# SimLeek/pySILEnT

Hardware: AMD Instinct MI355X
Metric: Mpx/s full pyramid line-end pass @1080p, 1/2/4/8 GPU; % HBM roofline (higher is better)
Workload: dtype f32

## Files before the change

### pysilent_amd/csrc/silent_rgb2.h

```cpp
#pragma once

#include "silent_rgb.h"

namespace silent {

typedef float f2 __attribute__((ext_vector_type(2)));
typedef unsigned long long u64;
typedef const __attribute__((address_space(4))) u64* ku64_p;

constexpr int kRgb2Halo = 8;
constexpr int kRgb2Cols = 128 - 2 * kRgb2Halo;
#ifndef RGB2_WAVES
#define RGB2_WAVES 2
#endif
constexpr int kRgb2Waves = RGB2_WAVES;
constexpr int kRgb2TW = kRgb2Waves * kRgb2Cols;
constexpr int kRgb2RowHalo = 7;
#ifndef RGB2_STORE_AUX
#define RGB2_STORE_AUX 2
#endif
constexpr int kRgb2StoreAux = RGB2_STORE_AUX;
constexpr int kRgb2Out = 0x40000000;

constexpr int kRgb2Blk = 16;
constexpr int kRgb2StreamMax = SILENT_RGB_STREAM_MAX;

constexpr int rgb2_popc(unsigned v) { return v ? (int)(v & 1u) + rgb2_popc(v >> 1) : 0; }

struct RgbSym {
    float rgc[12];
    float rgby[27];
};
constexpr int kSymRgc = 12, kSymRgby = 27, kSymStripe = 48;

template <unsigned RGC_PAIRS, bool STRIPE_SUM, bool RGBY_TWO, bool END_TWO, bool SYM = false>
struct Rgb2Layout {
    static constexpr int n_rgc = SYM ? kSymRgc : 9 * rgb2_popc(RGC_PAIRS & 0x1ffu);
    static constexpr int n_rgby = SYM ? kSymRgby : RGBY_TWO ? 45 : 81;
    static constexpr int n_stripe = SYM ? kSymStripe : STRIPE_SUM ? 27 : 81;
    static constexpr bool blur_sym = RGBY_TWO && END_TWO;
    static constexpr int n_blur = blur_sym ? 16 : 49;
    static constexpr int n_end = END_TWO ? 45 : 81;
    static constexpr int b_rgc = 0, b_rgby = b_rgc + n_rgc, b_stripe = (b_rgby + n_rgby + (SYM ? 1 : 0)) & ~(SYM ? 1 : 0),
                         b_blur = b_stripe + n_stripe, b_end = b_blur + n_blur, total = b_end + n_end;
    static constexpr int blocks = ((total + 2 * kRgb2Blk - 1) / (2 * kRgb2Blk)) * 2;
    static_assert(!SYM || (STRIPE_SUM && RGBY_TWO && END_TWO), "the symmetric forms extend the two-group instantiation");
};

constexpr int rgb2_conv_pos(unsigned pairs, int o, int dy, int dx, int i) {
    const unsigned row = (pairs >> (o * 3)) & 7u;
    const int before = 9 * rgb2_popc(pairs & ((1u << (o * 3)) - 1u));
    const int rank = dx * rgb2_popc(row) + rgb2_popc(row & ((1u << i) - 1u));
    return before + rank * 3 + (2 - dy);
}
inline int rgb2_fill_stream(const RgbW& w, unsigned rgc_pairs, bool stripe_sum, bool rgby_two, bool end_two, float* out,
                            const RgbSym* sym = nullptr) {
    const bool blur_sym = rgby_two && end_two;
    int n = 0;
    auto conv = [&](const float* k, unsigned pairs) {
        const int base = n;
        for (int o = 0; o < 3; ++o)
            for (int dy = 0; dy < 3; ++dy)
                for (int dx = 0; dx < 3; ++dx)
                    for (int i = 0; i < 3; ++i)
                        if ((pairs >> (o * 3 + i)) & 1u) {
                            out[base + rgb2_conv_pos(pairs, o, dy, dx, i)] = k[((o * 3 + dy) * 3 + dx) * 3 + i];
                            ++n;
                        }
    };
    auto two = [&](const float* k) {
        for (int j = 0; j < 9; ++j)
            for (int dy = 0; dy < 3; ++dy) out[n + j * 3 + (2 - dy)] = k[dy * 9 + j];
        for (int t = 0; t < 18; ++t) out[n + 27 + t] = k[27 + t];
        n += 45;
    };
    if (sym) {
        for (int c = 0; c < 3; ++c) {
            out[n + 0 + c] = sym->rgc[c * 4 + 0];
            out[n + 3 + c] = sym->rgc[c * 4 + 2];
            out[n + 6 + c] = sym->rgc[c * 4 + 1];
            out[n + 9 + c] = sym->rgc[c * 4 + 3];
        }
        n += kSymRgc;
        for (int t = 0; t < 9; ++t) out[n + t] = sym->rgby[t];
        for (int o = 0; o < 3; ++o) {
            out[n + 9 + o] = sym->rgby[9 + 0];
            out[n + 12 + o] = sym->rgby[9 + 3];
            out[n + 15 + o] = sym->rgby[9 + 1];
        }
        for (int t = 0; t < 9; ++t) out[n + 18 + t] = sym->rgby[18 + t];
        n += kSymRgby;
        if (n & 1) out[n++] = 0.0f;
        for (int o = 0; o < 3; ++o) {
            for (int dy = 0; dy < 3; ++dy) {
                const float l = w.stripe[((o * 3 + dy) * 3 + 0) * 3], c = w.stripe[((o * 3 + dy) * 3 + 1) * 3], r = w.stripe[((o * 3 + dy) * 3 + 2) * 3];
                out[n + (2 - dy) * 2] = l;
                out[n + (2 - dy) * 2 + 1] = r;
                out[n + 6 + (2 - dy)] = c;
                out[n + 10 + (2 - dy) * 2] = r;
                out[n + 10 + (2 - dy) * 2 + 1] = l;
            }
            out[n + 9] = 0.0f;
            n += 16;
        }
    } else {
    conv(w.rgc, rgc_pairs & 0x1ffu);
    if (rgby_two) two(w.rgby);
    else conv(w.rgby, 0x1ffu);
    if (stripe_sum) {
        for (int o = 0; o < 3; ++o)
            for (int dx = 0; dx < 3; ++dx)
                for (int dy = 0; dy < 3; ++dy) out[n + o * 9 + dx * 3 + (2 - dy)] = w.stripe[((o * 3 + dy) * 3 + dx) * 3];
        n += 27;
    } else {
        conv(w.stripe, 0x1ffu);
    }
    }
    if (blur_sym) {
        for (int j = 0; j < 4; ++j)
            for (int d = 0; d < 4; ++d) out[n + j * 4 + d] = w.blur[(3 + d) * 7 + j];
        n += 16;
    } else {
        for (int dx = 0; dx < 7; ++dx)
            for (int k = 0; k < 7; ++k) out[n + dx * 7 + k] = w.blur[(6 - k) * 7 + dx];
        n += 49;
    }
    if (end_two) two(w.end);
    else conv(w.end, 0x1ffu);
    const int total = n;
    while (n % (2 * kRgb2Blk)) out[n++] = 0.0f;
    return total;
}

struct Rgb2Args {
    const float* pyr;
    float* orient_out;
    float* line_out;
    float* value_out;
    LevelTab tab;
    RgbP prm;
    int th;
    unsigned* mm;
    float* sum;
    int* nan_flags;
    long long sum_frame;
    long long sum_off[kMaxLevels];
    alignas(64) float ws[kRgb2StreamMax];
};
static_assert(offsetof(Rgb2Args, ws) % 64 == 0, "weight blocks are whole 64-byte lines of the kernarg segment");

template <int NP>
struct WPairs {
    u64 p[NP];
};
__device__ __forceinline__ void wait_weights() { __builtin_amdgcn_s_waitcnt(0xC07F); }

template <int NB>
struct WStream {
    WPairs<kRgb2Blk / 2> A, B;
    ku64_p wp;
    template <int BLK>
    __device__ __forceinline__ void request() {
        ku64_p q = wp;
        __builtin_amdgcn_sched_barrier(0);
        asm volatile("" : "+s"(q));
        if constexpr (BLK & 1) {
#pragma unroll
            for (int k = 0; k < kRgb2Blk / 2; ++k) B.p[k] = q[BLK * (kRgb2Blk / 2) + k];
        } else {
#pragma unroll
            for (int k = 0; k < kRgb2Blk / 2; ++k) A.p[k] = q[BLK * (kRgb2Blk / 2) + k];
        }
    }
    template <int IDX>
    __device__ __forceinline__ u64 pair() {
        constexpr int blk = IDX / kRgb2Blk;
        if constexpr (IDX % kRgb2Blk == 0) {
            wait_weights();
            request<(blk + 1) % NB>();
        }
        if constexpr (blk & 1) return B.p[(IDX % kRgb2Blk) / 2];
        else return A.p[(IDX % kRgb2Blk) / 2];
    }
    template <int IDX>
    __device__ __forceinline__ f2 fma(const f2& x, const f2& c) {
        const u64 w = pair<IDX>();
        f2 r;
        if constexpr ((IDX & 1) == 0) asm volatile("v_pk_fma_f32 %0, %1, %2, %3 op_sel_hi:[1,0,1]" : "=v"(r) : "v"(x), "s"(w), "v"(c));
        else asm volatile("v_pk_fma_f32 %0, %1, %2, %3 op_sel:[0,1,0] op_sel_hi:[1,1,1]" : "=v"(r) : "v"(x), "s"(w), "v"(c));
        return r;
    }
    template <int IDX>
    __device__ __forceinline__ f2 fma0(const f2& x) {
        const u64 w = pair<IDX>();
        f2 r;
        if constexpr ((IDX & 1) == 0) asm volatile("v_pk_fma_f32 %0, %1, %2, 0 op_sel_hi:[1,0,0]" : "=v"(r) : "v"(x), "s"(w));
        else asm volatile("v_pk_fma_f32 %0, %1, %2, 0 op_sel:[0,1,0] op_sel_hi:[1,1,0]" : "=v"(r) : "v"(x), "s"(w));
        return r;
    }
    template <int IDX>
    __device__ __forceinline__ f2 mul(const f2& x) {
        const u64 w = pair<IDX>();
        f2 r;
        if constexpr ((IDX & 1) == 0) asm volatile("v_pk_mul_f32 %0, %1, %2 op_sel_hi:[1,0]" : "=v"(r) : "v"(x), "s"(w));
        else asm volatile("v_pk_mul_f32 %0, %1, %2 op_sel:[0,1] op_sel_hi:[1,1]" : "=v"(r) : "v"(x), "s"(w));
        return r;
    }
    template <int IDX>
    __device__ __forceinline__ f2 fma_sw(const f2& x, const f2& c) {
        static_assert((IDX & 1) == 0, "an aligned SGPR pair");
        const u64 w = pair<IDX>();
        f2 r;
        asm volatile("v_pk_fma_f32 %0, %1, %2, %3 op_sel:[1,0,0] op_sel_hi:[0,1,1]" : "=v"(r) : "v"(x), "s"(w), "v"(c));
        return r;
    }
    template <int IDX>
    __device__ __forceinline__ f2 fma0_sw(const f2& x) {
        static_assert((IDX & 1) == 0, "an aligned SGPR pair");
        const u64 w = pair<IDX>();
        f2 r;
        asm volatile("v_pk_fma_f32 %0, %1, %2, 0 op_sel:[1,0,0] op_sel_hi:[0,1,0]" : "=v"(r) : "v"(x), "s"(w));
        return r;
    }
    template <int FROM, int TO>
    __device__ __forceinline__ void skip() {
        if constexpr (FROM < TO) {
            constexpr int nb = (FROM + kRgb2Blk - 1) / kRgb2Blk * kRgb2Blk;
            if constexpr (nb < TO) {
                (void)pair<nb>();
                skip<nb + 1, TO>();
            }
        }
    }
};

template <int I>
using ic = std::integral_constant<int, I>;
template <int B, int E, class F>
__device__ __forceinline__ void rgb2_for(F&& f) {
    if constexpr (B < E) {
        f(ic<B>{});
        rgb2_for<B + 1, E>(f);
    }
}

__device__ __forceinline__ void neighbours2(const f2& c, f2& l, f2& r) {
    l.x = from_lane_below(c.y);
    l.y = c.x;
    r.x = c.y;
    r.y = from_lane_above(c.x);
}

__device__ __forceinline__ f2 side_pair(const f2& c) { return f2{from_lane_above(c.x), from_lane_below(c.y)}; }
__device__ __forceinline__ f2 pk_add_swap_both(const f2& a, const f2& b) {
    f2 r;
    asm("v_pk_add_f32 %0, %1, %2 op_sel:[1,1] op_sel_hi:[0,0]" : "=v"(r) : "v"(a), "v"(b));
    return r;
}
__device__ __forceinline__ f2 pk_add_swap_second(const f2& a, const f2& b) {
    f2 r;
    asm("v_pk_add_f32 %0, %1, %2 op_sel:[0,1] op_sel_hi:[1,0]" : "=v"(r) : "v"(a), "v"(b));
    return r;
}
__device__ __forceinline__ float relu_clip_max3(float v, float hi) {
    float r;
    asm("v_maximum3_f32 %0, %1, 0, 0" : "=v"(r) : "v"(v));
    asm("v_minimum3_f32 %0, %1, %2, %2" : "=v"(r) : "v"(r), "s"(hi));
    return r;
}

template <unsigned PAIRS, int BASE, class WS>
__device__ __forceinline__ void conv3_roll2(const f2 (&v)[3][3], WS& ws, f2 (&pa)[3], f2 (&pb)[3], f2 (&done)[3]) {
    f2 npa[3], npb[3];
    rgb2_for<0, 3>([&](auto oo) {
        constexpr int o = decltype(oo)::value;
        constexpr unsigned row = (PAIRS >> (o * 3)) & 7u;
        f2 t2 = pa[o], t1 = pb[o], t0 = f2{0.0f, 0.0f};
        if constexpr (row != 0) {
            constexpr int first_i = (row & 1u) ? 0 : ((row & 2u) ? 1 : 2);
            rgb2_for<0, 9>([&](auto jj) {
                constexpr int j = decltype(jj)::value, dx = j / 3, i = j % 3;
                if constexpr ((row >> i) & 1u) {
                    constexpr int p2 = BASE + rgb2_conv_pos(PAIRS, o, 2, dx, i);
                    t2 = ws.template fma<p2>(v[dx][i], t2);
                    t1 = ws.template fma<p2 + 1>(v[dx][i], t1);
                    if constexpr (dx == 0 && i == first_i) t0 = ws.template fma0<p2 + 2>(v[dx][i]);
                    else t0 = ws.template fma<p2 + 2>(v[dx][i], t0);
                }
            });
        }
        done[o] = t2;
        npa[o] = t1;
        npb[o] = t0;
    });
#pragma unroll
    for (int o = 0; o < 3; ++o) {
        pa[o] = npa[o];
        pb[o] = npb[o];
    }
}

template <unsigned M0, unsigned M1, unsigned M2, int BASE, class WS>
__device__ __forceinline__ void conv3_roll2_struct(const f2 (&v)[3][3], WS& ws, f2 (&pa)[6], f2 (&pb)[6], f2 (&done)[3]) {
    constexpr unsigned M[3] = {M0, M1, M2};
    f2 acc2[6], acc1[6], acc0[6];
#pragma unroll
    for (int q = 0; q < 6; ++q) {
        acc2[q] = pa[q];
        acc1[q] = pb[q];
        acc0[q] = f2{0.0f, 0.0f};
    }
    rgb2_for<0, 9>([&](auto jj) {
        constexpr int j = decltype(jj)::value, dx = j / 3, i = j % 3;
        constexpr int p = BASE + j * 3;
        constexpr int q2 = ((M[i] >> (2 * 3 + dx)) & 1u) ? i : 3 + i;
        constexpr int q1 = ((M[i] >> (1 * 3 + dx)) & 1u) ? i : 3 + i;
        constexpr bool a0 = (M[i] >> dx) & 1u;
        constexpr int q0 = a0 ? i : 3 + i;
        acc2[q2] = ws.template fma<p>(v[dx][i], acc2[q2]);
        acc1[q1] = ws.template fma<p + 1>(v[dx][i], acc1[q1]);
        constexpr unsigned taps = M[i] & 7u;
        constexpr bool seen = (dx >= 1 && (((taps >> 0) & 1u) != 0) == a0) || (dx >= 2 && (((taps >> 1) & 1u) != 0) == a0);
        if constexpr (!seen) acc0[q0] = ws.template fma0<p + 2>(v[dx][i]);
        else acc0[q0] = ws.template fma<p + 2>(v[dx][i], acc0[q0]);
    });
    {
        constexpr int PM = BASE + 27;
        f2 t[3];
        rgb2_for<0, 3>([&](auto oo) {
            constexpr int o = decltype(oo)::value;
            t[o] = ws.template mul<PM + o>(acc2[0]);
        });
        rgb2_for<1, 6>([&](auto kk) {
            constexpr int k = decltype(kk)::value;
            rgb2_for<0, 3>([&](auto oo) {
                constexpr int o = decltype(oo)::value;
                t[o] = ws.template fma<PM + k * 3 + o>(acc2[k], t[o]);
            });
        });
#pragma unroll
        for (int o = 0; o < 3; ++o) done[o] = t[o];
    }
#pragma unroll
    for (int q = 0; q < 6; ++q) {
        pa[q] = acc1[q];
        pb[q] = acc0[q];
    }
}

template <int BASE, class WS>
__device__ __forceinline__ void conv3_roll2_sum(const f2 (&s)[3], WS& ws, f2 (&pa)[3], f2 (&pb)[3], f2 (&done)[3]) {
    f2 npa[3], npb[3];
    rgb2_for<0, 3>([&](auto oo) {
        constexpr int o = decltype(oo)::value;
        f2 t2 = pa[o], t1 = pb[o], t0;
        rgb2_for<0, 3>([&](auto xx) {
            constexpr int dx = decltype(xx)::value, p = BASE + o * 9 + dx * 3;
            t2 = ws.template fma<p>(s[dx], t2);
            t1 = ws.template fma<p + 1>(s[dx], t1);
            if constexpr (dx == 0) t0 = ws.template fma0<p + 2>(s[dx]);
            else t0 = ws.template fma<p + 2>(s[dx], t0);
        });
        done[o] = t2;
        npa[o] = t1;
        npb[o] = t0;
    });
#pragma unroll
    for (int o = 0; o < 3; ++o) {
        pa[o] = npa[o];
        pb[o] = npb[o];
    }
}

__device__ __forceinline__ float relu_ok(float v, bool ok) { return ok ? relu_tf(v) : 0.0f; }
__device__ __forceinline__ float relu_max3(float v) {
    float r;
    asm("v_maximum3_f32 %0, %1, 0, 0" : "=v"(r) : "v"(v));
    return r;
}
__device__ __forceinline__ float relu_max3_poisoned(float v, float u) {
    float r;
    asm("v_maximum3_f32 %0, %1, 0, %2" : "=v"(r) : "v"(v), "v"(u));
    return r;
}

typedef _Float16 rgb_half;
template <unsigned RGC_PAIRS, bool STRIPE_SUM, unsigned RGBY_A, unsigned END_A0, unsigned END_A1, unsigned END_A2, bool MM = false, bool SYM = false,
          bool ST4 = false, typename ST = float>
__global__ __launch_bounds__(64 * kRgb2Waves) __attribute__((amdgpu_waves_per_eu((MM || ST4) ? 3 : 4, 8))) void rgb_line_end2_kernel(const Rgb2Args args) {
    typedef Rgb2Layout<RGC_PAIRS, STRIPE_SUM, RGBY_A != kDense, END_A0 != kDense, SYM> L;
    constexpr bool kHalf = std::is_same<ST, rgb_half>::value;
    static_assert(kHalf || std::is_same<ST, float>::value, "orient / line_end are stored as float32 or float16");
    static_assert(!(kHalf && ST4), "ST4 is a float32 store form");
    static_assert(L::blocks * kRgb2Blk <= kRgb2StreamMax, "stream fits its kernarg array");
    static_assert((RGC_PAIRS & 0x1ffu) == 0x1ffu || (RGC_PAIRS & 0x1ffu) == 0x111u, "rgc: dense or channel-diagonal");
    constexpr bool kRgcDiag = (RGC_PAIRS & 0x1ffu) == 0x111u;
    const int R = args.th, NROWS = R + 2 * kRgb2RowHalo;
    const float* __restrict__ pyr = args.pyr;
    float* __restrict__ orient_out = args.orient_out;
    float* __restrict__ line_out = args.line_out;
    float* __restrict__ value_out = args.value_out;
    const LevelTab& tab = args.tab;
    const RgbP& prm = args.prm;

    typedef const __attribute__((address_space(4))) char* kchar_p;
    WStream<L::blocks> ws;
    ws.wp = (ku64_p)((kchar_p)__builtin_amdgcn_kernarg_segment_ptr() + offsetof(Rgb2Args, ws));
    ws.template request<0>();

    const TileCoord tc = locate_tile(tab, blockIdx.x);
    const int H = tab.h[tc.level], W = tab.w[tc.level];
    const long long base_px = (long long)tc.frame * tab.frame_px + tab.px_off[tc.level];
    const float* __restrict__ src = pyr + base_px * 3;
    const int lane = threadIdx.x & 63;
    const int wave = __builtin_amdgcn_readfirstlane(threadIdx.x >> 6);
    const int xw0 = tc.tx * kRgb2TW + wave * kRgb2Cols;
    if (xw0 >= W) return;
    const int y0 = tc.ty * R;
    const int x0 = xw0 + 2 * lane - kRgb2Halo, x1 = x0 + 1;
    const bool col0 = x0 >= 0 && x0 < W, col1 = x1 >= 0 && x1 < W;
    const bool out_lane = lane >= kRgb2Halo / 2 && lane < 64 - kRgb2Halo / 2;
    const bool out0 = out_lane && x0 < W, out1 = out_lane && x1 < W;
    const int rb = W * 12;
    const int rows_t = R < H - y0 ? R : H - y0;
    const unsigned lvl_bytes = (unsigned)H * (unsigned)rb;
    const unsigned tile_bytes = (unsigned)rows_t * (unsigned)rb;
    const long long tile_px = base_px + (long long)y0 * W;
    const __amdgpu_buffer_rsrc_t r_src = __builtin_amdgcn_make_buffer_rsrc((void*)src, 0, lvl_bytes, 0x00020000);
    __amdgpu_buffer_rsrc_t r_orient = __builtin_amdgcn_make_buffer_rsrc((void*)(orient_out + tile_px * 3), 0, orient_out ? tile_bytes : 0u, 0x00020000);
    __amdgpu_buffer_rsrc_t r_line = __builtin_amdgcn_make_buffer_rsrc((void*)(line_out + tile_px * 3), 0, line_out ? tile_bytes : 0u, 0x00020000);
    unsigned mis_o = 0, mis_l = 0;
    if constexpr (kHalf) {
        auto half_rsrc = [&](float* p, unsigned& mis) {
            const unsigned long long b = reinterpret_cast<unsigned long long>(p) + (unsigned long long)(tile_px * 6);
            mis = (unsigned)__builtin_amdgcn_readfirstlane((int)(b & 2ull));
            return __builtin_amdgcn_make_buffer_rsrc((void*)(b - mis), 0, p ? tile_bytes / 2u + mis : 0u, 0x00020000);
        };
        r_orient = half_rsrc(orient_out, mis_o);
        r_line = half_rsrc(line_out, mis_l);
    }
    const __amdgpu_buffer_rsrc_t r_value = __builtin_amdgcn_make_buffer_rsrc((void*)(value_out + tile_px), 0, value_out ? tile_bytes / 3u : 0u, 0x00020000);
    const int in0 = col0 ? x0 * 12 : kRgb2Out, in1 = col1 ? x1 * 12 : kRgb2Out;
    const int xa = xw0 - kRgb2Halo + lane, xb = xa + 64;
    const int sta = (lane >= kRgb2Halo && xa < W) ? xa * 12 : kRgb2Out, stb = (lane < 64 - kRgb2Halo && xb < W) ? xb * 12 : kRgb2Out;
    const int sv2 = (out0 && out1) ? x0 * 4 : kRgb2Out, sv1 = (out0 && !out1) ? x0 * 4 : kRgb2Out;
    const bool padc0 = x0 >= prm.pad && x0 < W - prm.pad, padc1 = x1 >= prm.pad && x1 < W - prm.pad;
    const f2 inv3p = {1.0f / 3.0f, 1.0f / 3.0f};
    const f2 zero2 = {0.0f, 0.0f};

    f2 a1[3] = {zero2, zero2, zero2}, b1[3] = {zero2, zero2, zero2};
    f2 a2[6] = {zero2, zero2, zero2, zero2, zero2, zero2}, b2[6] = {zero2, zero2, zero2, zero2, zero2, zero2};
    f2 a3[3] = {zero2, zero2, zero2}, b3[3] = {zero2, zero2, zero2};
    f2 a5[6] = {zero2, zero2, zero2, zero2, zero2, zero2}, b5[6] = {zero2, zero2, zero2, zero2, zero2, zero2};
    f2 pb[7] = {zero2, zero2, zero2, zero2, zero2, zero2, zero2};
    __shared__ f2 s_hist[kRgb2Waves][4][3][64];
    float mm_mx = kPoolLowest, mm_nmn = kPoolLowest;
    float mm_grp = kPoolLowest;
    unsigned long long mm_nan = 0;
    const int gpt = (R + kSumRows - 1) / kSumRows, nxp = (W + 1) >> 1;
    const unsigned sum_bytes = (MM && args.sum) ? (unsigned)((rows_t + kSumRows - 1) / kSumRows) * (unsigned)nxp * 4u : 0u;
    const __amdgpu_buffer_rsrc_t r_sum = __builtin_amdgcn_make_buffer_rsrc(
        (void*)(args.sum + (long long)tc.frame * args.sum_frame + args.sum_off[tc.level] + (long long)tc.ty * gpt * nxp), 0, sum_bytes, 0x00020000);
    const int ssum = out0 ? (x0 >> 1) * 4 : kRgb2Out;
    __shared__ __attribute__((aligned(16))) float s_tr[kRgb2Waves][ST4 ? 4 * 384 : kHalf ? 1 : 384];
    float* const tr = s_tr[wave];
    typedef int i3 __attribute__((ext_vector_type(3)));
    f2* const tr_in = reinterpret_cast<f2*>(tr) + lane * 3;
    const float* const tr_out = tr + (lane >> 1) * 6 + (lane & 1);
    auto store_row3 = [&](const f2 (&val)[3], __amdgpu_buffer_rsrc_t rsrc, int ro) {
#pragma unroll
        for (int c = 0; c < 3; ++c) tr_in[c] = val[c];
        const i3 da = {__float_as_int(tr_out[0]), __float_as_int(tr_out[2]), __float_as_int(tr_out[4])};
        const i3 db = {__float_as_int(tr_out[192]), __float_as_int(tr_out[194]), __float_as_int(tr_out[196])};
        __builtin_amdgcn_raw_buffer_store_b96(da, rsrc, (int)((unsigned)sta + (unsigned)ro), 0, kRgb2StoreAux);
        __builtin_amdgcn_raw_buffer_store_b96(db, rsrc, (int)((unsigned)stb + (unsigned)ro), 0, kRgb2StoreAux);
    };
    const int hb = x0 * 6;
    const bool h_two = out0 && out1, h_one = out0 && !out1;
    const bool h_next = lane + 1 < 64 - kRgb2Halo / 2 && x0 + 2 < W;
    const bool h_lead = lane == kRgb2Halo / 2 - 1;
    const int he96 = h_two ? hb : kRgb2Out, ho96 = (h_two && h_next) ? hb + 2 : kRgb2Out;
    const int ho64 = (h_two && !h_next) ? hb + 2 : kRgb2Out;
    const int h32 = h_one ? hb : kRgb2Out;
    const int he16 = h_one ? hb + 4 : kRgb2Out;
    const int ho16 = h_lead ? hb + 12 : (h_two && !h_next) ? hb + 10 : kRgb2Out;
    const unsigned lead_sh = h_lead ? 16u : 0u;
    auto store_row3h = [&](const f2 (&val)[3], __amdgpu_buffer_rsrc_t rsrc, unsigned ro) {
        typedef rgb_half h2 __attribute__((ext_vector_type(2)));
        typedef int i2h __attribute__((ext_vector_type(2)));
        const int d0 = __builtin_bit_cast(int, h2{(rgb_half)val[0].x, (rgb_half)val[1].x});
        const int d1 = __builtin_bit_cast(int, h2{(rgb_half)val[2].x, (rgb_half)val[0].y});
        const int d2 = __builtin_bit_cast(int, h2{(rgb_half)val[1].y, (rgb_half)val[2].y});
        int m = -(int)((ro >> 1) & 1u);
        asm volatile("" : "+s"(m));
        auto pick = [&](int even, int odd) { return (odd & m) | (even & ~m); };
        const unsigned sh = (unsigned)(m & 16);
        const int up = __builtin_amdgcn_update_dpp(0, d0, 0x130 , 0xf, 0xf, true);
        const int e0 = (int)__builtin_amdgcn_alignbit((unsigned)d1, (unsigned)d0, sh);
        const int e1 = (int)__builtin_amdgcn_alignbit((unsigned)d2, (unsigned)d1, sh);
        const int e2 = (int)__builtin_amdgcn_alignbit((unsigned)up, (unsigned)d2, sh);
        const int last = pick(e1, (int)((unsigned)e2 >> lead_sh));
        __builtin_amdgcn_raw_buffer_store_b96(i3{e0, e1, e2}, rsrc, (int)((unsigned)pick(he96, ho96) + ro), 0, kRgb2StoreAux);
        __builtin_amdgcn_raw_buffer_store_b64(i2h{e0, e1}, rsrc, (int)((unsigned)pick(kRgb2Out, ho64) + ro), 0, kRgb2StoreAux);
        __builtin_amdgcn_raw_buffer_store_b32(e0, rsrc, (int)((unsigned)h32 + (ro + (unsigned)(m & 2))), 0, kRgb2StoreAux);
        __builtin_amdgcn_raw_buffer_store_b16((short)last, rsrc, (int)((unsigned)pick(he16, ho16) + ro), 0, kRgb2StoreAux);
    };
    auto row_off_h = [&](int k, unsigned mis) {
        const int norow = (k | (rows_t - 1 - k)) >> 31;
        return norow != 0 ? (unsigned)kRgb2Out : mis + (unsigned)(k * (W * 6));
    };
    typedef int i4v __attribute__((ext_vector_type(4)));
    int st4_off[3] = {0, 0, 0}, st4_lds[3] = {0, 0, 0};
    if constexpr (ST4) {
        const int colb = (xw0 - kRgb2Halo) * 12;
        const int wend = (xw0 + kRgb2Cols < W ? xw0 + kRgb2Cols : W);
        auto chunk = [&](int q, int rowb, int ldsb, int& off, int& lds) {
            const int x_last = xw0 - kRgb2Halo + (4 * q + 3) / 3;
            const bool ok = q >= 6 && q < 90 && x_last < wend;
            off = ok ? rowb + colb + 16 * q : kRgb2Out;
            lds = ldsb + 16 * (q < 96 ? q : 95);
        };
        chunk(6 + lane, 0, 0, st4_off[0], st4_lds[0]);
        if (lane < 20) chunk(70 + lane, 0, 0, st4_off[1], st4_lds[1]);
        else chunk(lane - 14, rb, 1536, st4_off[1], st4_lds[1]);
        chunk(lane < 40 ? 50 + lane : 95, rb, 1536, st4_off[2], st4_lds[2]);
        if (lane >= 40) st4_off[2] = kRgb2Out;
    }
    auto st4_put = [&](const f2 (&val)[3], int m, int slot) {
        float* const dst = tr + (m * 2 + slot) * 384 + lane * 6;
#pragma unroll
        for (int c = 0; c < 3; ++c) {
            dst[c] = val[c].x;
            dst[3 + c] = val[c].y;
        }
    };
    auto st4_flush = [&](int m, __amdgpu_buffer_rsrc_t rsrc, int roA) {
        const char* const base = reinterpret_cast<const char*>(tr + m * 2 * 384);
#pragma unroll
        for (int k = 0; k < 3; ++k) {
            const i4v d = *reinterpret_cast<const i4v*>(base + st4_lds[k]);
            __builtin_amdgcn_raw_buffer_store_b128(d, rsrc, (int)((unsigned)st4_off[k] + (unsigned)roA), 0, kRgb2StoreAux);
        }
    };
#pragma unroll
    for (int k = 0; k < 4; ++k)
#pragma unroll
        for (int c = 0; c < 3; ++c) s_hist[wave][k][c][lane] = zero2;

    i3 nb0[2], nb1[2];
    auto fetch = [&](i3 (&buf)[2], int row) {
        const unsigned ro = (unsigned)((y0 - kRgb2RowHalo + row) * rb);
        buf[0] = __builtin_amdgcn_raw_buffer_load_b96(r_src, (int)((unsigned)in0 + ro), 0, 0);
        buf[1] = __builtin_amdgcn_raw_buffer_load_b96(r_src, (int)((unsigned)in1 + ro), 0, 0);
    };
    fetch(nb0, 0);
    fetch(nb1, 1);
#pragma unroll
    for (int k = 0; k < (MM ? 14 : 12) + (kHalf ? 8 : 0); ++k) __builtin_amdgcn_raw_buffer_store_b32(k, r_value, kRgb2Out + 64 * k, 0, 0);

    const bool cols_ok = __builtin_amdgcn_readfirstlane(__all(col0 && col1 && padc0 && padc1) ? 1 : 0) != 0;
    const int in_hi = (H - prm.pad < H - 6 ? H - prm.pad : H - 6) - prm.pad;
    const unsigned in_len = (cols_ok && in_hi > 0) ? (unsigned)in_hi : 0u;
    auto mask_stage = [&](f2 (&g)[3], int y, int outside) {
        if (outside != 0) {
            const bool rok = (unsigned)y < (unsigned)H;
#pragma unroll
            for (int c = 0; c < 3; ++c) g[c] = f2{(rok && col0) ? g[c].x : 0.0f, (rok && col1) ? g[c].y : 0.0f};
        }
    };
    auto relu_stage = [&](f2 (&g)[3], int y, int outside) {
        if constexpr (SYM) {
#pragma unroll
            for (int c = 0; c < 3; ++c) g[c] = f2{relu_max3(g[c].x), relu_max3(g[c].y)};
        } else {
#pragma unroll
            for (int c = 0; c < 3; ++c) g[c] = f2{relu_tf(g[c].x), relu_tf(g[c].y)};
        }
        mask_stage(g, y, outside);
    };
    auto step = [&](int row, i3 (&mine)[2], auto parity) {
        constexpr int PAR = decltype(parity)::value;
        const int yin = y0 - kRgb2RowHalo + row;
        const int outside = ((yin - 7 - prm.pad) | ((int)in_len - 1 - (yin - 7 - prm.pad))) >> 31;
        f2 v[3][3], g[3];
#pragma unroll
        for (int c = 0; c < 3; ++c) {
            v[1][c] = f2{__int_as_float(mine[0][c]), __int_as_float(mine[1][c])};
        }
        asm volatile("" : "+v"(v[1][0]), "+v"(v[1][1]), "+v"(v[1][2]));
        fetch(mine, row + 2);
        if constexpr (SYM) {
            f2 F[3], E[3], M[3];
#pragma unroll
            for (int c = 0; c < 3; ++c) F[c] = pk_add_swap_both(side_pair(v[1][c]), v[1][c]);
            rgb2_for<0, 3>([&](auto cc) { constexpr int c = decltype(cc)::value; E[c] = ws.template mul<L::b_rgc + c>(F[c]); });
            rgb2_for<0, 3>([&](auto cc) { constexpr int c = decltype(cc)::value; M[c] = ws.template fma<L::b_rgc + 3 + c>(F[c], b1[c]); });
            rgb2_for<0, 3>([&](auto cc) { constexpr int c = decltype(cc)::value; E[c] = ws.template fma<L::b_rgc + 6 + c>(v[1][c], E[c]); });
            rgb2_for<0, 3>([&](auto cc) { constexpr int c = decltype(cc)::value; M[c] = ws.template fma<L::b_rgc + 9 + c>(v[1][c], M[c]); });
#pragma unroll
            for (int c = 0; c < 3; ++c) {
                g[c] = a1[c] + E[c];
                a1[c] = M[c];
                b1[c] = E[c];
            }
        } else {
#pragma unroll
            for (int c = 0; c < 3; ++c) neighbours2(v[1][c], v[0][c], v[2][c]);
            conv3_roll2<RGC_PAIRS & 0x1ffu, L::b_rgc>(v, ws, a1, b1, g);
        }
        {
            if constexpr (kRgcDiag) {
                const f2 sg = (g[0] + g[1]) + g[2];
                const f2 u = sg - sg;
                if constexpr (SYM) {
#pragma unroll
                    for (int c = 0; c < 3; ++c) g[c] = f2{relu_max3_poisoned(g[c].x, u.x), relu_max3_poisoned(g[c].y, u.y)};
                } else {
#pragma unroll
                    for (int c = 0; c < 3; ++c) g[c] = g[c] + u;
#pragma unroll
                    for (int c = 0; c < 3; ++c) g[c] = f2{relu_tf(g[c].x), relu_tf(g[c].y)};
                }
                mask_stage(g, yin - 1, outside);
            } else {
                relu_stage(g, yin - 1, outside);
            }
        }
        if constexpr (SYM) {
            constexpr int B = L::b_rgby;
            f2 Z[3], F[3], E[3], M[3];
            rgb2_for<0, 9>([&](auto tt) {
                constexpr int t = decltype(tt)::value, i = t / 3, o = t % 3;
                if constexpr (i == 0) Z[o] = ws.template mul<B + t>(g[0]);
                else Z[o] = ws.template fma<B + t>(g[i], Z[o]);
            });
#pragma unroll
            for (int o = 0; o < 3; ++o) F[o] = pk_add_swap_both(side_pair(Z[o]), Z[o]);
            rgb2_for<0, 3>([&](auto oo) { constexpr int o = decltype(oo)::value; E[o] = ws.template mul<B + 9 + o>(F[o]); });
            rgb2_for<0, 3>([&](auto oo) { constexpr int o = decltype(oo)::value; M[o] = ws.template fma<B + 12 + o>(F[o], b2[o]); });
            rgb2_for<0, 3>([&](auto oo) { constexpr int o = decltype(oo)::value; E[o] = ws.template fma<B + 15 + o>(Z[o], E[o]); });
            rgb2_for<0, 9>([&](auto tt) {
                constexpr int t = decltype(tt)::value, i = t / 3, o = t % 3;
                M[o] = ws.template fma<B + 18 + t>(g[i], M[o]);
            });
#pragma unroll
            for (int o = 0; o < 3; ++o) {
                g[o] = a2[o] + E[o];
                a2[o] = M[o];
                b2[o] = E[o];
            }
        } else {
#pragma unroll
        for (int c = 0; c < 3; ++c) {
            v[1][c] = g[c];
            neighbours2(v[1][c], v[0][c], v[2][c]);
        }
        if constexpr (RGBY_A != kDense) conv3_roll2_struct<RGBY_A, RGBY_A, RGBY_A, L::b_rgby>(v, ws, a2, b2, g);
        else conv3_roll2<0x1ffu, L::b_rgby>(v, ws, reinterpret_cast<f2 (&)[3]>(a2), reinterpret_cast<f2 (&)[3]>(b2), g);
        }
        {
            relu_stage(g, yin - 2, outside);
        }
        if constexpr (SYM) {
            const f2 S = (g[0] + g[1]) + g[2];
            const f2 D = side_pair(S);
            f2 npa[3], npb[3];
            rgb2_for<0, 3>([&](auto oo) {
                constexpr int o = decltype(oo)::value, B = L::b_stripe + o * 16;
                f2 t2 = a3[o], t1 = b3[o], t0;
                t2 = ws.template fma_sw<B + 0>(D, t2);
                t1 = ws.template fma_sw<B + 2>(D, t1);
                t0 = ws.template fma0_sw<B + 4>(D);
                t2 = ws.template fma<B + 6>(S, t2);
                t1 = ws.template fma<B + 7>(S, t1);
                t0 = ws.template fma<B + 8>(S, t0);
                t2 = ws.template fma_sw<B + 10>(S, t2);
                t1 = ws.template fma_sw<B + 12>(S, t1);
                t0 = ws.template fma_sw<B + 14>(S, t0);
                g[o] = t2;
                npa[o] = t1;
                npb[o] = t0;
            });
#pragma unroll
            for (int o = 0; o < 3; ++o) {
                a3[o] = npa[o];
                b3[o] = npb[o];
            }
        } else if constexpr (STRIPE_SUM) {
            f2 s3[3];
            s3[1] = (g[0] + g[1]) + g[2];
            neighbours2(s3[1], s3[0], s3[2]);
            conv3_roll2_sum<L::b_stripe>(s3, ws, a3, b3, g);
        } else {
#pragma unroll
            for (int c = 0; c < 3; ++c) {
                v[1][c] = g[c];
                neighbours2(v[1][c], v[0][c], v[2][c]);
            }
            conv3_roll2<0x1ffu, L::b_stripe>(v, ws, a3, b3, g);
        }
        {
            relu_stage(g, yin - 3, outside);
        }
        f2 xs3[3];
#pragma unroll
        for (int c = 0; c < 3; ++c) {
            s_hist[wave][row & 3][c][lane] = g[c];
            xs3[c] = s_hist[wave][(row + 1) & 3][c][lane];
        }
        f2 bdone;
        {
            const f2 s = (g[0] + g[1]) + g[2];
            f2 T[7];
            f2 nb[7];
            if constexpr (SYM) {
                const f2 X = side_pair(s);
                const f2 Y = f2{from_lane_below(s.x), from_lane_above(s.y)};
                const f2 Q = f2{from_lane_below(X.y), from_lane_above(X.x)};
                T[0] = pk_add_swap_second(Q, Y);
                T[1] = Y + X;
                T[2] = pk_add_swap_both(X, s);
                T[3] = s;
            } else {
            const float a = from_lane_below(s.x), b = from_lane_below(s.y), c = from_lane_above(s.x), d = from_lane_above(s.y);
            const float e = from_lane_below(b), f = from_lane_above(c);
            T[0] = f2{e, a};
            T[1] = f2{a, b};
            T[2] = f2{b, s.x};
            T[3] = s;
            T[4] = f2{s.y, c};
            T[5] = f2{c, d};
            T[6] = f2{d, f};
            }
            if constexpr (L::blur_sym) {
                f2 F[4];
                if constexpr (SYM) {
#pragma unroll
                    for (int j = 0; j < 4; ++j) F[j] = T[j];
                } else {
                    F[0] = T[0] + T[6];
                    F[1] = T[1] + T[5];
                    F[2] = T[2] + T[4];
                    F[3] = T[3];
                }
                f2 P[4];
                rgb2_for<0, 4>([&](auto jj) {
                    constexpr int j = decltype(jj)::value;
                    rgb2_for<0, 4>([&](auto dd) {
                        constexpr int d = decltype(dd)::value, p = L::b_blur + j * 4 + d;
                        if constexpr (j == 0) P[d] = ws.template mul<p>(F[0]);
                        else P[d] = ws.template fma<p>(F[j], P[d]);
                    });
                });
                nb[0] = pb[0] + P[3];
                nb[1] = pb[1] + P[2];
                nb[2] = pb[2] + P[1];
                nb[3] = pb[3] + P[0];
                nb[4] = pb[4] + P[1];
                nb[5] = pb[5] + P[2];
                nb[6] = P[3];
            } else {
            rgb2_for<0, 7>([&](auto xx) {
                constexpr int dx = decltype(xx)::value;
                rgb2_for<0, 7>([&](auto kk) {
                    constexpr int k = decltype(kk)::value, p = L::b_blur + dx * 7 + k;
                    if constexpr (dx == 0) {
                        if constexpr (k == 6) nb[k] = ws.template fma0<p>(T[0]);
                        else nb[k] = ws.template fma<p>(T[0], pb[k]);
                    } else {
                        nb[k] = ws.template fma<p>(T[dx], nb[k]);
                    }
                });
            });
            }
            bdone = nb[0];
#pragma unroll
            for (int k = 0; k < 6; ++k) pb[k] = nb[k + 1];
        }
        const int t = yin - 6;
        f2 o3[3];
        {
            f2 rr;
            if constexpr (SYM) {
                float m0, m1;
                asm("v_minimum3_f32 %0, %1, 1.0, 1.0" : "=v"(m0) : "v"(bdone.x));
                asm("v_minimum3_f32 %0, %1, 1.0, 1.0" : "=v"(m1) : "v"(bdone.y));
                rr = f2{prm.rv * __builtin_amdgcn_exp2f(-prm.root * __builtin_amdgcn_logf(m0)),
                        prm.rv * __builtin_amdgcn_exp2f(-prm.root * __builtin_amdgcn_logf(m1))};
                const bool s0 = (m0 > 0.0f && m0 < 7.8886e-31f) || prm.root == 0.0f, s1 = (m1 > 0.0f && m1 < 7.8886e-31f) || prm.root == 0.0f;
                if (s0 || s1) {
                    if (s0) rr.x = prm.rv / powf(m0, prm.root);
                    if (s1) rr.y = prm.rv / powf(m1, prm.root);
                }
            } else {
                rr = f2{regulator_ratio(bdone.x, prm.rv, prm.root), regulator_ratio(bdone.y, prm.rv, prm.root)};
            }
            int flat_policy = prm.flat_policy;
            asm volatile("" : "+s"(flat_policy));
#pragma unroll
            for (int c = 0; c < 3; ++c) {
                const f2 xs = xs3[c];
                f2 y = xs * rr;
                if (flat_policy == SILENT_FLAT_ZERO) {
                    if (xs.x == 0.0f) y.x = 0.0f;
                    if (xs.y == 0.0f) y.y = 0.0f;
                }
                o3[c] = y;
            }
            if (outside != 0) {
                const bool rok = (unsigned)t < (unsigned)H;
#pragma unroll
                for (int c = 0; c < 3; ++c) o3[c] = f2{(rok && col0) ? o3[c].x : 0.0f, (rok && col1) ? o3[c].y : 0.0f};
            }
        }
        if constexpr (ST4) {
            st4_put(o3, 0, PAR == 1 ? 0 : 1);
            if constexpr (PAR == 0) st4_flush(0, r_orient, (t - y0 - 1) * rb);
        } else if constexpr (kHalf) {
            store_row3h(o3, r_orient, row_off_h(t - y0, mis_o));
        } else {
            store_row3(o3, r_orient, (t - y0) * rb);
        }
#pragma unroll
        for (int c = 0; c < 3; ++c) {
            v[1][c] = o3[c];
            neighbours2(v[1][c], v[0][c], v[2][c]);
        }
        if constexpr (END_A0 != kDense) conv3_roll2_struct<END_A0, END_A1, END_A2, L::b_end>(v, ws, a5, b5, g);
        else conv3_roll2<0x1ffu, L::b_end>(v, ws, reinterpret_cast<f2 (&)[3]>(a5), reinterpret_cast<f2 (&)[3]>(b5), g);
        const int yout = yin - 7, k = yout - y0;
        {
            f2 le[3];
#pragma unroll
            for (int c = 0; c < 3; ++c)
                le[c] = SYM ? f2{relu_clip_max3(g[c].x, prm.clip_hi), relu_clip_max3(g[c].y, prm.clip_hi)}
                            : f2{clip_hi_tf(relu_tf(g[c].x), prm.clip_hi), clip_hi_tf(relu_tf(g[c].y), prm.clip_hi)};
            if (outside != 0) {
                const bool padr = yout >= prm.pad && yout < H - prm.pad;
                const f2 mk = {(padc0 && padr) ? 1.0f : 0.0f, (padc1 && padr) ? 1.0f : 0.0f};
#pragma unroll
                for (int c = 0; c < 3; ++c) le[c] = mk * le[c];
            }
            if constexpr (ST4) {
                st4_put(le, 1, PAR == 0 ? 0 : 1);
                if constexpr (PAR == 1) st4_flush(1, r_line, (k - 1) * rb);
            } else if constexpr (kHalf) {
                store_row3h(le, r_line, row_off_h(k, mis_l));
            } else {
                store_row3(le, r_line, k * rb);
            }
            const f2 val = ((le[0] + le[1]) + le[2]) * inv3p;
            typedef int i2 __attribute__((ext_vector_type(2)));
            const int norow = (k | (rows_t - 1 - k)) >> 31;
            if (MM && norow == 0) {
                const float a = out0 ? val.x : kPoolLowest, b = out1 ? val.y : kPoolLowest;
                const float na = out0 ? -val.x : kPoolLowest, nb = out1 ? -val.y : kPoolLowest;
                asm("v_max3_f32 %0, %1, %2, %3" : "=v"(mm_mx) : "v"(mm_mx), "v"(a), "v"(b));
                asm("v_max3_f32 %0, %1, %2, %3" : "=v"(mm_nmn) : "v"(mm_nmn), "v"(na), "v"(nb));
                asm("v_max3_f32 %0, %1, %2, %3" : "=v"(mm_grp) : "v"(mm_grp), "v"(a), "v"(b));
                mm_nan |= __ballot((out0 && val.x != val.x) || (out1 && val.y != val.y));
            }
            if constexpr (MM) {
                const bool gend = norow == 0 && (((k + 1) & (kSumRows - 1)) == 0 || k == rows_t - 1);
                const unsigned so = gend ? (unsigned)((k >> kSumRowsLog2) * nxp * 4) : (unsigned)kRgb2Out;
                __builtin_amdgcn_raw_buffer_store_b32(__float_as_int(mm_grp), r_sum, (int)((unsigned)ssum + so), 0, 0);
                mm_grp = gend ? kPoolLowest : mm_grp;
            }
            const unsigned rv = (unsigned)(k * W * 4);
            __builtin_amdgcn_raw_buffer_store_b64(i2{__float_as_int(val.x), __float_as_int(val.y)}, r_value, (int)((unsigned)sv2 + rv), 0, 0);
            __builtin_amdgcn_raw_buffer_store_b32(__float_as_int(val.x), r_value, (int)((unsigned)sv1 + rv), 0, 0);
        }
        ws.template skip<L::total, L::blocks * kRgb2Blk>();
    };
#pragma unroll 1
    for (int row = 0; row < NROWS; row += 2) {
        step(row, nb0, ic<0>{});
        step(row + 1, nb1, ic<1>{});
    }
    if constexpr (MM) {
        const float mx = wave_max(mm_mx), nmn = wave_max(mm_nmn);
        if (lane == 0) {
            unsigned* slot = args.mm + ((long long)tc.frame * tab.n_levels + tc.level) * 2;
            atomicMax(slot, f2ord(mx));
            atomicMax(slot + 1, f2ord(nmn));
            if (mm_nan && args.nan_flags) args.nan_flags[tc.frame * tab.n_levels + tc.level] = 1;
        }
    }
}

}
```

Before: 142,500.

## Split row loop into warm-up phases that skip stages not yet needed

The row loop is split into three phases. Early halo rows run only up to the stripe stage, the next rows run up to the blur, and only later rows run the regulator/end stage and issue stores. This is meant to avoid computing outputs for halo rows that were previously thrown away, at the cost of three copies of the step body (larger code) and a new weight-stream finish path that has to keep the SGPR weight pipeline in sync.

```diff
diff --git a/pysilent_amd/csrc/silent_rgb2.h b/pysilent_amd/csrc/silent_rgb2.h
--- a/pysilent_amd/csrc/silent_rgb2.h
+++ b/pysilent_amd/csrc/silent_rgb2.h
@@ -21,6 +21,23 @@
 #endif
 constexpr int kRgb2StoreAux = RGB2_STORE_AUX;
 constexpr int kRgb2Out = 0x40000000;
+
+constexpr int kRgb2Lag3x3 = 1, kRgb2LagBlur = 3;
+constexpr int kRgb2LagStripe = 3 * kRgb2Lag3x3;
+constexpr int kRgb2LagReg = kRgb2LagStripe + kRgb2LagBlur;
+constexpr int kRgb2LagEnd = kRgb2LagReg + kRgb2Lag3x3;
+constexpr int kRgb2NeedReg = kRgb2RowHalo - kRgb2Lag3x3;
+constexpr int kRgb2NeedStripe = kRgb2NeedReg - kRgb2LagBlur;
+constexpr int kRgb2FirstFull = kRgb2NeedReg + kRgb2LagReg;
+constexpr int kRgb2FirstBlur = kRgb2NeedStripe + kRgb2LagStripe;
+constexpr int kRgb2FirstStripe = kRgb2FirstBlur - 2 * kRgb2Lag3x3;
+enum : int { kRgb2ToStripe = 0, kRgb2ToBlur = 1, kRgb2Full = 2 };
+static_assert(kRgb2LagEnd == kRgb2RowHalo, "the five stages consume the row halo");
+static_assert(kRgb2FirstFull == 2 * kRgb2RowHalo - 2 * kRgb2Lag3x3, "the end bank takes two rows before the one that completes output row 0");
+static_assert(kRgb2FirstBlur == kRgb2FirstFull - 2 * kRgb2LagBlur, "the blur takes six rows before the one that completes a row");
+static_assert(kRgb2FirstStripe >= 0 && kRgb2FirstBlur > 0, "the short steps exist");
+static_assert(kRgb2FirstBlur % 2 == 0 && kRgb2FirstFull % 2 == 0, "phases are whole pairs of rows: nb0 / nb1, the row pairs of ST4, the stripe ring");
+static_assert(kRgb2FirstFull < 2 + 2 * kRgb2RowHalo, "the smallest tile (two rows) still runs full steps");
 
 constexpr int kRgb2Blk = 16;
 constexpr int kRgb2StreamMax = SILENT_RGB_STREAM_MAX;
@@ -230,6 +247,16 @@
                 (void)pair<nb>();
                 skip<nb + 1, TO>();
             }
+        }
+    }
+    template <int FROM>
+    __device__ __forceinline__ void finish() {
+        constexpr int lb = (FROM - 1) / kRgb2Blk;
+        if constexpr (lb + 2 >= NB) {
+            skip<FROM, NB * kRgb2Blk>();
+        } else {
+            if constexpr (((lb + 1) & 1) == 0) wait_weights();
+            request<0>();
         }
     }
 };
@@ -555,8 +582,6 @@
     };
     fetch(nb0, 0);
     fetch(nb1, 1);
-#pragma unroll
-    for (int k = 0; k < (MM ? 14 : 12) + (kHalf ? 8 : 0); ++k) __builtin_amdgcn_raw_buffer_store_b32(k, r_value, kRgb2Out + 64 * k, 0, 0);
 
     const bool cols_ok = __builtin_amdgcn_readfirstlane(__all(col0 && col1 && padc0 && padc1) ? 1 : 0) != 0;
     const int in_hi = (H - prm.pad < H - 6 ? H - prm.pad : H - 6) - prm.pad;
@@ -578,8 +603,9 @@
         }
         mask_stage(g, y, outside);
     };
-    auto step = [&](int row, i3 (&mine)[2], auto parity) {
+    auto step = [&](int row, i3 (&mine)[2], auto parity, auto last) {
         constexpr int PAR = decltype(parity)::value;
+        constexpr int LAST = decltype(last)::value;
         const int yin = y0 - kRgb2RowHalo + row;
         const int outside = ((yin - 7 - prm.pad) | ((int)in_len - 1 - (yin - 7 - prm.pad))) >> 31;
         f2 v[3][3], g[3];
@@ -706,7 +732,11 @@
 #pragma unroll
         for (int c = 0; c < 3; ++c) {
             s_hist[wave][row & 3][c][lane] = g[c];
-            xs3[c] = s_hist[wave][(row + 1) & 3][c][lane];
+            if constexpr (LAST == kRgb2Full) xs3[c] = s_hist[wave][(row + 1) & 3][c][lane];
+        }
+        if constexpr (LAST == kRgb2ToStripe) {
+            ws.template finish<L::b_blur>();
+            return;
         }
         f2 bdone;
         {
@@ -777,6 +807,10 @@
 #pragma unroll
             for (int k = 0; k < 6; ++k) pb[k] = nb[k + 1];
         }
+        if constexpr (LAST == kRgb2ToBlur) {
+            ws.template finish<L::b_end>();
+            return;
+        }
         const int t = yin - 6;
         f2 o3[3];
         {
@@ -870,12 +904,25 @@
             __builtin_amdgcn_raw_buffer_store_b64(i2{__float_as_int(val.x), __float_as_int(val.y)}, r_value, (int)((unsigned)sv2 + rv), 0, 0);
             __builtin_amdgcn_raw_buffer_store_b32(__float_as_int(val.x), r_value, (int)((unsigned)sv1 + rv), 0, 0);
         }
-        ws.template skip<L::total, L::blocks * kRgb2Blk>();
-    };
+        ws.template finish<L::total>();
+    };
+    int row = 0;
 #pragma unroll 1
-    for (int row = 0; row < NROWS; row += 2) {
-        step(row, nb0, ic<0>{});
-        step(row + 1, nb1, ic<1>{});
+    for (; row < kRgb2FirstBlur; row += 2) {
+        step(row, nb0, ic<0>{}, ic<kRgb2ToStripe>{});
+        step(row + 1, nb1, ic<1>{}, ic<kRgb2ToStripe>{});
+    }
+#pragma unroll 1
+    for (; row < kRgb2FirstFull; row += 2) {
+        step(row, nb0, ic<0>{}, ic<kRgb2ToBlur>{});
+        step(row + 1, nb1, ic<1>{}, ic<kRgb2ToBlur>{});
+    }
+#pragma unroll
+    for (int k = 0; k < (MM ? 14 : 12) + (kHalf ? 8 : 0); ++k) __builtin_amdgcn_raw_buffer_store_b32(k, r_value, kRgb2Out + 64 * k, 0, 0);
+#pragma unroll 1
+    for (; row < NROWS; row += 2) {
+        step(row, nb0, ic<0>{}, ic<kRgb2Full>{});
+        step(row + 1, nb1, ic<1>{}, ic<kRgb2Full>{});
     }
     if constexpr (MM) {
         const float mx = wave_max(mm_mx), nmn = wave_max(mm_nmn);
```

Result: no change. 142,400 (-0.1%).
